# rhymes-ai/Aria

Measured on NVIDIA H100. Metric: Aria-25.3B bf16 prefill tokens/sec, higher is better.
Workload: dtype bf16

## Files before the change

### aria_b200/csrc/gemm.cu

```cuda
#include <cuda_fp8.h>

#include "gemm_common.cuh"

namespace aria {

constexpr int GEMM_STAGES = 4;
constexpr int FP8_LAND_STAGES = 3;
constexpr int FP8_CONVERT_WARPS = 3;
constexpr int PAIR_MIN_ROWS = 2048;
template <int BN, bool B_FP8 = false>
constexpr int gemm_smem_bytes() {
  return 1024  + GEMM_STAGES * (A_STAGE_BYTES + BN * BK * 2) + BM * acc_ld(BN) * 4 + 256  +
         (B_FP8 ? FP8_LAND_STAGES * BN * BK : 0);
}
static_assert(gemm_smem_bytes<128, true>() <= 232448, "fp8 landing ring must fit the opt-in shared memory of a block");

ARIA_DEVICE void e4m3x16_to_bf16(const uint4 v, uint4& lo, uint4& hi) {
  const uint32_t w[4] = {v.x, v.y, v.z, v.w};
  uint32_t o[8];
#pragma unroll
  for (int i = 0; i < 4; ++i) {
#pragma unroll
    for (int h = 0; h < 2; ++h) {
      const __half2_raw hr = __nv_cvt_fp8x2_to_halfraw2(static_cast<__nv_fp8x2_storage_t>(w[i] >> (16 * h)), __NV_E4M3);
      const float2 f = __half22float2(__half2(hr));
      o[2 * i + h] = pack_bf16(f.x, f.y);
    }
  }
  lo = make_uint4(o[0], o[1], o[2], o[3]);
  hi = make_uint4(o[4], o[5], o[6], o[7]);
}

template <bool PAIR> ARIA_DEVICE int first_tile() { return PAIR ? blockIdx.x >> 1 : blockIdx.x; }
template <bool PAIR> ARIA_DEVICE int tile_step() { return PAIR ? gridDim.x >> 1 : gridDim.x; }
template <bool PAIR> ARIA_DEVICE int pair_sched_n(int n_tiles) { return PAIR ? (n_tiles + 1) / 2 : n_tiles; }

template <int BN, bool B_MN>
ARIA_DEVICE void wgmma_tile_k16(float (&acc)[BN / 2], uint64_t da, uint64_t db) {
  if constexpr (BN == 128) wgmma_m64n128_ss<0, B_MN ? 1 : 0>(acc, da, db, 1u);
  else wgmma_m64n144_ss<0, B_MN ? 1 : 0>(acc, da, db, 1u);
}

template <int BN, bool B_MN, int EPI, bool B_FP8 = false, bool PAIR = false>
__global__ void __launch_bounds__(GEMM_THREADS, 1)
gemm_kernel(const __grid_constant__ CUtensorMap tmA, const __grid_constant__ CUtensorMap tmB0,
            const __grid_constant__ CUtensorMap tmB1, const __grid_constant__ CUtensorMap tmB2, const GemmParams p) {
  constexpr int B_STAGE_BYTES = BN * BK * 2;
  constexpr int STAGE_BYTES = A_STAGE_BYTES + B_STAGE_BYTES;
  constexpr int STAGES = GEMM_STAGES;
  constexpr int ACC_LD = acc_ld(BN);
  constexpr int OUT_BN = (EPI == ARIA_EPI_SWIGLU) ? BN / 2 : BN;
  static_assert(BN == 128 || BN == 144, "tile widths with a wgmma wrapper");
  static_assert(!B_FP8 || (B_MN && BN == 128 && EPI != ARIA_EPI_HEADS), "fp8 B: grouped [G, K, N] weights, 128-wide tiles");
  static_assert(!PAIR || (!B_MN && !B_FP8), "CTA pairs: dense K-major bf16 B");
  constexpr int LAND_BYTES = BN * BK;

  uint8_t* smem = smem_1024();
  float* stg = reinterpret_cast<float*>(smem + STAGES * STAGE_BYTES);
  const BarrierRing<STAGES> bar(stg + BM * ACC_LD);
  const BarrierRing<FP8_LAND_STAGES> land_bar(bar.empty + STAGES);
  uint8_t* land = reinterpret_cast<uint8_t*>(bar.full) + 256;

  const int warp = threadIdx.x >> 5;
  const int lane = threadIdx.x & 31;
  const int wg = threadIdx.x >> 7;

  if (warp == 0 && lane == 0) {
    prefetch_tmap(&tmA);
    prefetch_tmap(&tmB0);
    if (p.n_seg > 1 || EPI == ARIA_EPI_SWIGLU) prefetch_tmap(&tmB1);
    if (p.n_seg > 2) prefetch_tmap(&tmB2);
    bar.init(B_FP8 ? 1 + FP8_CONVERT_WARPS : 1, PAIR ? 2 * CONSUMER_WARPS : CONSUMER_WARPS);
    if constexpr (B_FP8) land_bar.init(1, FP8_CONVERT_WARPS);
    fence_mbar_init();
  }
  if constexpr (PAIR) cluster_sync();
  else __syncthreads();

  const int n_out_total = p.N * (EPI == ARIA_EPI_SWIGLU ? 1 : p.n_seg);
  const int n_tiles = (n_out_total + OUT_BN - 1) / OUT_BN;
  const int k_blocks = (p.K + BK - 1) / BK;
  const uint32_t smem_base = smem_u32(smem);
  const uint32_t full0 = smem_u32(bar.full), empty0 = smem_u32(bar.empty);

  if (wg == 0) {
    setmaxnreg_dec<40>();
    if (warp == 0 && elect_one()) {
      const uint32_t rank = PAIR ? cluster_ctarank() : 0;
      TileSched sched;
      sched.init(p, pair_sched_n<PAIR>(n_tiles));
      RingPos<STAGES> rp;
      RingPos<FP8_LAND_STAGES> lp;
      for (int t = first_tile<PAIR>();; t += tile_step<PAIR>()) {
        int grp, m_idx, n_idx, row0, rows;
        if (!sched.decode(t, grp, m_idx, n_idx, row0, rows)) break;
        if constexpr (PAIR) n_idx = 2 * n_idx + rank;
        const bool phantom = PAIR && n_idx >= n_tiles;
        const int a_row = row0 + m_idx * BM;
        const int a_half_row = a_row + (m_idx * BM + static_cast<int>(rank) * (BM / 2) < rows ? rank * (BM / 2) : 0);
        const int bgrp = weight_block(p, grp);
        int b_c0 = 0, b_c1 = 0;
        const CUtensorMap* tb0 = &tmB0;
        const CUtensorMap* tb1 = &tmB1;
        if constexpr (B_MN) {
          b_c0 = bgrp * p.K;
        } else if constexpr (EPI == ARIA_EPI_SWIGLU) {
          b_c0 = b_c1 = n_idx * OUT_BN;
        } else {
          const int col = n_idx * BN;
          const int seg = col / p.N;
          tb0 = seg == 0 ? &tmB0 : (seg == 1 ? &tmB1 : &tmB2);
          b_c0 = col - seg * p.N + bgrp * p.b_group_rows;
        }
        for (int kb = 0; kb < k_blocks; ++kb) {
          const uint32_t fb = full0 + rp.stage * 8;
          const uint32_t sa = smem_base + rp.stage * STAGE_BYTES;
          const uint32_t sb = sa + A_STAGE_BYTES;
          mbar_wait_addr(empty0 + rp.stage * 8, rp.phase ^ 1);
          if constexpr (PAIR) {
            mbar_arrive_expect_tx_addr(fb, phantom ? A_STAGE_BYTES : STAGE_BYTES);
            tma_load_2d_multicast_addr(sa + rank * (A_STAGE_BYTES / 2), &tmA, fb, kb * BK, a_half_row, 0b11);
            if (phantom) {
              rp.next();
              continue;
            }
          } else {
            mbar_arrive_expect_tx_addr(fb, B_FP8 ? A_STAGE_BYTES : STAGE_BYTES);
            tma_load_2d_addr(sa, &tmA, fb, kb * BK, a_row);
          }
          if constexpr (B_MN) {
            uint32_t dst = sb, box_bytes = 64 * BK * 2, bar_addr = fb;
            if constexpr (B_FP8) {
              bar_addr = smem_u32(land_bar.full) + lp.stage * 8;
              mbar_wait_addr(smem_u32(land_bar.empty) + lp.stage * 8, lp.phase ^ 1);
              mbar_arrive_expect_tx_addr(bar_addr, LAND_BYTES);
              dst = smem_u32(land) + lp.stage * LAND_BYTES;
              box_bytes = 64 * BK;
            }
            const int krow = b_c0 + kb * BK;
#pragma unroll
            for (int c = 0; c < BN / 64; ++c)
              tma_load_2d_addr(dst + c * box_bytes, &tmB0, bar_addr, tile_b_col<BN, EPI>(c * 64, n_idx, p.N), krow);
            if constexpr (B_FP8) lp.next();
          } else if constexpr (EPI == ARIA_EPI_SWIGLU) {
            tma_load_2d_addr(sb, tb0, fb, kb * BK, b_c0);
            tma_load_2d_addr(sb + (BN / 2) * BK * 2, tb1, fb, kb * BK, b_c1);
          } else {
            tma_load_2d_addr(sb, tb0, fb, kb * BK, b_c0);
          }
          rp.next();
        }
      }
    } else if constexpr (B_FP8) {
      if (warp > 0) {
        const int ct = threadIdx.x - 32;
        TileSched sched;
        sched.init(p, n_tiles);
        RingPos<STAGES> rp;
        RingPos<FP8_LAND_STAGES> lp;
        for (int t = blockIdx.x;; t += gridDim.x) {
          int grp, m_idx, n_idx, row0, rows;
          if (!sched.decode(t, grp, m_idx, n_idx, row0, rows)) break;
          for (int kb = 0; kb < k_blocks; ++kb) {
            mbar_wait_addr(smem_u32(land_bar.full) + lp.stage * 8, lp.phase);
            const uint8_t* src = land + lp.stage * LAND_BYTES;
            uint8_t* dst = smem + rp.stage * STAGE_BYTES + A_STAGE_BYTES;
#pragma unroll 1
            for (int i = ct; i < LAND_BYTES / 16; i += FP8_CONVERT_WARPS * 32) {
              const uint4 v = *reinterpret_cast<const uint4*>(src + i * 16);
              uint4 lo, hi;
              e4m3x16_to_bf16(v, lo, hi);
              const int r = (i >> 2) & 63, j = 2 * (i & 3);
              uint8_t* row = dst + (i >> 8) * (64 * BK * 2) + r * 128;
              *reinterpret_cast<uint4*>(row + ((j ^ (r & 7)) << 4)) = lo;
              *reinterpret_cast<uint4*>(row + (((j + 1) ^ (r & 7)) << 4)) = hi;
            }
            fence_proxy_async_smem();
            __syncwarp();
            if (lane == 0) {
              mbar_arrive(&bar.full[rp.stage]);
              mbar_arrive(&land_bar.empty[lp.stage]);
            }
            rp.next();
            lp.next();
          }
        }
      }
    }
  } else {
    setmaxnreg_inc<232>();
    const int cw = wg - 1;
    constexpr uint32_t b_lbo = B_MN ? 64 * BK * 2 : 16;
    constexpr uint32_t b_sbo = 1024;
    constexpr uint32_t b_kadv = (B_MN ? 16 * 128 : 32) >> 4;
    const uint64_t da0 = make_smem_desc(smem_base + cw * 64 * 128, 16, 1024);
    const uint64_t db0 = make_smem_desc(smem_base + A_STAGE_BYTES, b_lbo, b_sbo);
    const ConsumerThread ct = consumer_thread(cw, lane);
    const uint32_t rank = PAIR ? cluster_ctarank() : 0;
    TileSched sched;
    sched.init(p, pair_sched_n<PAIR>(n_tiles));
    RingPos<STAGES> rp;
    auto release = [&](int s) {
      if (lane == 0) {
        mbar_arrive(&bar.empty[s]);
        if constexpr (PAIR) mbar_arrive_cluster(&bar.empty[s], rank ^ 1);
      }
    };
    for (int t = first_tile<PAIR>();; t += tile_step<PAIR>()) {
      int grp, m_idx, n_idx, row0, rows;
      if (!sched.decode(t, grp, m_idx, n_idx, row0, rows)) break;
      if constexpr (PAIR) {
        n_idx = 2 * n_idx + rank;
        if (n_idx >= n_tiles) {
          for (int kb = 0; kb < k_blocks; ++kb) {
            mbar_wait_addr(full0 + rp.stage * 8, rp.phase);
            release(rp.stage);
            rp.next();
          }
          continue;
        }
      }
      float acc[BN / 2];
#pragma unroll
      for (int i = 0; i < BN / 2; ++i) acc[i] = 0.f;
      float2 bsc[BN / 8];
      if constexpr (B_FP8) load_col_scales<BN, EPI>(p, grp, n_idx, ct.frag_col, bsc);
      int prev = -1;
      for (int kb = 0; kb < k_blocks; ++kb) {
        mbar_wait_addr(full0 + rp.stage * 8, rp.phase);
        const uint64_t da = da0 + rp.stage * (STAGE_BYTES >> 4);
        const uint64_t db = db0 + rp.stage * (STAGE_BYTES >> 4);
        wgmma_fence();
#pragma unroll
        for (int k = 0; k < BK / 16; ++k) wgmma_tile_k16<BN, B_MN>(acc, da + k * 2, db + k * b_kadv);
        wgmma_commit();
        wgmma_wait<1>();
        if (prev >= 0) release(prev);
        prev = static_cast<int>(rp.stage);
        rp.next();
      }
      wgmma_wait<0>();
      fence_regs(acc);
      if (prev >= 0) release(prev);
      stage_and_epilogue<BN, EPI, B_FP8 ? AccScale::COL : AccScale::NONE>(p, stg, ct, acc, bsc, 1.f, 1.f, n_out_total, grp,
                                                                           m_idx, n_idx, row0, rows);
    }
  }
  if constexpr (PAIR) cluster_sync();
}

constexpr int W8_BK = 128;
static_assert(BM * W8_BK == A_STAGE_BYTES, "W8A8 A stage = bf16 A stage");

template <int EPI>
__global__ void __launch_bounds__(GEMM_THREADS, 1)
gemm_w8a8_kernel(const __grid_constant__ CUtensorMap tmA, const __grid_constant__ CUtensorMap tmB, const GemmParams p,
                 const float* __restrict__ a_scale) {
  constexpr int BN = 128;
  constexpr int STAGE_BYTES = A_STAGE_BYTES + BN * W8_BK;
  constexpr int STAGES = GEMM_STAGES;
  constexpr int ACC_LD = acc_ld(BN);
  constexpr int OUT_BN = (EPI == ARIA_EPI_SWIGLU) ? BN / 2 : BN;
  static_assert(EPI == ARIA_EPI_LINEAR || EPI == ARIA_EPI_SWIGLU, "W8A8: expert GEMM epilogues");

  uint8_t* smem = smem_1024();
  float* stg = reinterpret_cast<float*>(smem + STAGES * STAGE_BYTES);
  const BarrierRing<STAGES> bar(stg + BM * ACC_LD);

  const int warp = threadIdx.x >> 5;
  const int lane = threadIdx.x & 31;
  const int wg = threadIdx.x >> 7;

  if (warp == 0 && lane == 0) {
    prefetch_tmap(&tmA);
    prefetch_tmap(&tmB);
    bar.init(1, CONSUMER_WARPS);
    fence_mbar_init();
  }
  __syncthreads();

  const int n_tiles = (p.N + OUT_BN - 1) / OUT_BN;
  const int k_blocks = p.K / W8_BK;
  const uint32_t smem_base = smem_u32(smem);
  const uint32_t full0 = smem_u32(bar.full), empty0 = smem_u32(bar.empty);

  if (wg == 0) {
    setmaxnreg_dec<40>();
    if (warp == 0 && elect_one()) {
      TileSched sched;
      sched.init(p, n_tiles);
      RingPos<STAGES> rp;
      for (int t = blockIdx.x;; t += gridDim.x) {
        int grp, m_idx, n_idx, row0, rows;
        if (!sched.decode(t, grp, m_idx, n_idx, row0, rows)) break;
        const int a_row = row0 + m_idx * BM;
        int b_r0, b_r1;
        if constexpr (EPI == ARIA_EPI_SWIGLU) {
          b_r0 = weight_block(p, grp) * 2 * p.N + n_idx * OUT_BN;
          b_r1 = b_r0 + p.N;
        } else {
          b_r0 = weight_block(p, grp) * p.N + n_idx * BN;
          b_r1 = b_r0 + 64;
        }
        for (int kb = 0; kb < k_blocks; ++kb) {
          const uint32_t fb = full0 + rp.stage * 8;
          const uint32_t sa = smem_base + rp.stage * STAGE_BYTES;
          const uint32_t sb = sa + A_STAGE_BYTES;
          mbar_wait_addr(empty0 + rp.stage * 8, rp.phase ^ 1);
          mbar_arrive_expect_tx_addr(fb, STAGE_BYTES);
          tma_load_2d_addr(sa, &tmA, fb, kb * W8_BK, a_row);
          tma_load_2d_addr(sb, &tmB, fb, kb * W8_BK, b_r0);
          tma_load_2d_addr(sb + 64 * W8_BK, &tmB, fb, kb * W8_BK, b_r1);
          rp.next();
        }
      }
    }
  } else {
    setmaxnreg_inc<232>();
    const int cw = wg - 1;
    const uint64_t da0 = make_smem_desc(smem_base + cw * 64 * 128, 16, 1024);
    const uint64_t db0 = make_smem_desc(smem_base + A_STAGE_BYTES, 16, 1024);
    const ConsumerThread ct = consumer_thread(cw, lane);
    TileSched sched;
    sched.init(p, n_tiles);
    RingPos<STAGES> rp;
    float part[BN / 2];
    for (int t = blockIdx.x;; t += gridDim.x) {
      int grp, m_idx, n_idx, row0, rows;
// ... 53 lines not shown
  p.ldo = d->ldo;
  p.head_dim = d->head_dim;
  p.head_ld = d->head_ld;
  p.rows_per_batch = d->rows_per_batch > 0 ? d->rows_per_batch : static_cast<int>(d->m);
  p.pos0 = d->pos0;
  p.stride_b = d->stride_b;
  p.stride_h = d->stride_h;
  p.rope_mask = d->rope_mask;
  p.rope_cos = static_cast<const __nv_bfloat16*>(d->rope_cos);
  p.rope_sin = static_cast<const __nv_bfloat16*>(d->rope_sin);
  p.position_ids = d->position_ids;
  p.b_scale = b_scale;
  return p;
}

static aria_gemm_desc_t grouped_desc(const void* a, const void* b, void* out, const int32_t* offsets, int64_t rows, int64_t k,
                                     int64_t n, int32_t groups, int32_t epilogue) {
  aria_gemm_desc_t d{};
  d.a = a;
  d.lda = k;
  d.m = rows;
  d.n = n;
  d.k = k;
  d.b[0] = b;
  d.n_seg = 1;
  d.b_layout = ARIA_B_GKN;
  d.num_groups = groups;
  d.group_offsets = offsets;
  d.epilogue = epilogue;
  d.out[0] = out;
  d.ldo = n;
  return d;
}

static int64_t max_tiles(const aria_gemm_desc_t* d, int BN, int64_t groups) {
  const bool swiglu = d->epilogue == ARIA_EPI_SWIGLU;
  const int out_bn = swiglu ? BN / 2 : BN;
  const int64_t n_out_total = d->n * (swiglu ? 1 : d->n_seg);
  return (n_out_total + out_bn - 1) / out_bn * ((d->m + BM - 1) / BM + groups);
}

static int gemm_run(const aria_gemm_desc_t* d, const float* b_scale, cudaStream_t stream) {
  ARIA_CHECK_ARG(d != nullptr);
  ARIA_CHECK_ARG(d->a && d->b[0] && d->out[0]);
  ARIA_CHECK_ARG(d->m >= 0 && d->n > 0 && d->k > 0);
  ARIA_CHECK_ARG(d->n % 8 == 0 && d->k % 8 == 0 && d->lda % 8 == 0);
  ARIA_CHECK_ARG(d->n_seg >= 1 && d->n_seg <= 3);
  ARIA_CHECK_ARG(d->num_groups >= 1 && (d->group_mod >= 0 || d->num_groups % (-d->group_mod) == 0));
  ARIA_CHECK_ARG((reinterpret_cast<uintptr_t>(d->a) & 15) == 0 && (reinterpret_cast<uintptr_t>(d->out[0]) & 15) == 0);
  if (d->m == 0) return ARIA_OK;
  const bool b_mn = d->b_layout == ARIA_B_GKN;
  const bool b_gnk = d->b_layout == ARIA_B_GNK;
  const bool swiglu = d->epilogue == ARIA_EPI_SWIGLU;
  if (b_mn) {
    ARIA_CHECK_ARG(d->n_seg == 1);
    ARIA_CHECK_ARG(d->k % BK == 0 || (d->num_groups == 1 && d->group_mod == 0));
    ARIA_CHECK_ARG(d->n % 64 == 0);
    ARIA_CHECK_ARG(d->epilogue != ARIA_EPI_HEADS);
  } else {
    ARIA_CHECK_ARG(d->num_groups == 1 || d->n_seg == 1);
    if (swiglu) ARIA_CHECK_ARG(d->n_seg == 2 && d->b[1]);
    if (b_gnk) ARIA_CHECK_ARG(d->n_seg == 1 && !swiglu && d->epilogue == ARIA_EPI_LINEAR && d->n % 128 == 0);
    else ARIA_CHECK_ARG(d->num_groups == 1);
  }
  if (d->num_groups > 1) ARIA_CHECK_ARG(d->group_offsets != nullptr);
  if (d->group_counts) ARIA_CHECK_ARG(d->group_offsets != nullptr);
  if (d->out_group_base) ARIA_CHECK_ARG(d->out_group_row0 != nullptr && d->epilogue == ARIA_EPI_LINEAR && d->group_offsets != nullptr);
  ARIA_CHECK_ARG(d->a_rows == 0 || d->a_rows >= d->m);

  int BN = 128;
  if (d->epilogue == ARIA_EPI_HEADS) {
    ARIA_CHECK_ARG(d->head_dim > 0 && d->head_dim % 8 == 0 && d->head_ld >= d->head_dim && d->n % d->head_dim == 0);
    if (d->rope_mask) ARIA_CHECK_ARG(d->head_dim == 128 && d->rope_cos && d->rope_sin);
    if (d->n % 128 != 0) {
      ARIA_CHECK_ARG(!d->rope_mask && d->n % 144 == 0);
      BN = 144;
    }
    for (int s = 0; s < d->n_seg; ++s) ARIA_CHECK_ARG(d->out[s] && d->b[s]);
  } else {
    if (swiglu) ARIA_CHECK_ARG(d->n % 64 == 0);
    if (d->n_seg > 1 && !swiglu) ARIA_CHECK_ARG(d->n % BN == 0);
  }

  const bool pair = !b_scale && d->b_layout == ARIA_B_NK && d->num_groups == 1 && !d->group_offsets &&
                    d->epilogue == ARIA_EPI_LINEAR && d->m >= PAIR_MIN_ROWS;

  CUtensorMap tmA, tmB[3];
  int rc = make_tmap_2d(&tmA, d->a, d->k, d->a_rows > 0 ? d->a_rows : d->m, d->lda * 2, BK, pair ? BM / 2 : BM);
  if (rc) return rc;
  if (b_mn) {
    const uint64_t ncols = swiglu ? 2 * d->n : d->n;
    const uint64_t n_weights = d->group_mod > 0 ? d->group_mod : (d->group_mod < 0 ? d->num_groups / (-d->group_mod) : d->num_groups);
    rc = b_scale ? make_tmap_2d(&tmB[0], d->b[0], ncols, n_weights * d->k, ncols, 64, BK, CU_TENSOR_MAP_SWIZZLE_NONE,
                                CU_TENSOR_MAP_DATA_TYPE_UINT8)
                 : make_tmap_2d(&tmB[0], d->b[0], ncols, n_weights * d->k, ncols * 2, 64, BK);
    if (rc) return rc;
    tmB[1] = tmB[0];
    tmB[2] = tmB[0];
  } else {
    const int nb = swiglu ? 2 : d->n_seg;
    const uint32_t box_rows = swiglu ? BN / 2 : BN;
    for (int s = 0; s < 3; ++s) {
      const void* ptr = s < nb ? d->b[s] : d->b[0];
      const uint64_t b_rows = b_gnk ? static_cast<uint64_t>(d->group_mod > 0 ? d->group_mod : (d->group_mod < 0 ? d->num_groups / (-d->group_mod) : d->num_groups)) * d->n : d->n;
      rc = make_tmap_2d(&tmB[s], ptr, d->k, b_rows, d->k * 2, BK, box_rows);
      if (rc) return rc;
    }
  }

  const GemmParams p = gemm_params(d, b_scale);
  const int64_t tiles = max_tiles(d, BN, d->num_groups > 1 ? d->num_groups : 0);
  if (pair) {
    const int64_t m_tiles = (d->m + BM - 1) / BM, pairs = (tiles / m_tiles + 1) / 2 * m_tiles;
    return launch_persistent_pairs<gemm_kernel<128, false, ARIA_EPI_LINEAR, false, true>>(
        "gemm_kernel", GEMM_THREADS, gemm_smem_bytes<128>(), pairs, stream, tmA, tmB[0], tmB[1], tmB[2], p);
  }
#define ARIA_LAUNCH(BN_, MN_, EPI_, ...)                                                                                     \
  return launch_persistent<gemm_kernel<BN_, MN_, EPI_, ##__VA_ARGS__>>("gemm_kernel", GEMM_THREADS,                          \
                                                                       gemm_smem_bytes<BN_, ##__VA_ARGS__>(), tiles, stream, \
                                                                       tmA, tmB[0], tmB[1], tmB[2], p)
  if (b_scale) {
    if (swiglu) ARIA_LAUNCH(128, true, ARIA_EPI_SWIGLU, true);
    ARIA_LAUNCH(128, true, ARIA_EPI_LINEAR, true);
  }
  if (d->epilogue == ARIA_EPI_HEADS) {
    if (BN == 128) ARIA_LAUNCH(128, false, ARIA_EPI_HEADS);
    ARIA_LAUNCH(144, false, ARIA_EPI_HEADS);
  }
  if (swiglu) {
    if (b_mn) ARIA_LAUNCH(128, true, ARIA_EPI_SWIGLU);
    ARIA_LAUNCH(128, false, ARIA_EPI_SWIGLU);
  }
  if (b_mn) ARIA_LAUNCH(128, true, ARIA_EPI_LINEAR);
  ARIA_LAUNCH(128, false, ARIA_EPI_LINEAR);
#undef ARIA_LAUNCH
}

extern "C" int aria_gemm(const aria_gemm_desc_t* d, aria_stream_t stream) {
  return gemm_run(d, nullptr, reinterpret_cast<cudaStream_t>(stream));
}

int aria::grouped_gemm(const void* a, const void* b, const float* b_scale, void* out, const int32_t* offsets, int64_t rows,
                       int64_t k, int64_t n, int32_t groups, int32_t epilogue, cudaStream_t stream) {
  const aria_gemm_desc_t d = grouped_desc(a, b, out, offsets, rows, k, n, groups, epilogue);
  return gemm_run(&d, b_scale, stream);
}

extern "C" int aria_grouped_gemm(const void* a, const void* b, void* out, const int32_t* group_offsets, int64_t rows,
                                 int64_t k, int64_t n, int32_t num_groups, aria_stream_t stream) {
  return grouped_gemm(a, b, nullptr, out, group_offsets, rows, k, n, num_groups, ARIA_EPI_LINEAR,
                      reinterpret_cast<cudaStream_t>(stream));
}

extern "C" int aria_grouped_gemm_fp8(const void* a, const void* b_fp8, const float* b_scale, void* out,
                                     const int32_t* group_offsets, int64_t rows, int64_t k, int64_t n, int32_t num_groups,
                                     int32_t epilogue, aria_stream_t stream) {
  ARIA_CHECK_ARG(a && b_fp8 && b_scale && out && group_offsets);
  ARIA_CHECK_ARG(rows >= 0 && k > 0 && n > 0 && k % BK == 0 && n % 64 == 0 && num_groups >= 1);
  ARIA_CHECK_ARG(epilogue == ARIA_EPI_LINEAR || epilogue == ARIA_EPI_SWIGLU);
  ARIA_CHECK_ARG((reinterpret_cast<uintptr_t>(a) & 15) == 0 && (reinterpret_cast<uintptr_t>(b_fp8) & 15) == 0 &&
                 (reinterpret_cast<uintptr_t>(b_scale) & 15) == 0 && (reinterpret_cast<uintptr_t>(out) & 15) == 0);
  return grouped_gemm(a, b_fp8, b_scale, out, group_offsets, rows, k, n, num_groups, epilogue,
                      reinterpret_cast<cudaStream_t>(stream));
}

extern "C" int aria_grouped_gemm_w8a8(const void* a_fp8, const float* a_scale, const void* b_fp8_nk, const float* b_scale,
                                      void* out, const int32_t* group_offsets, int64_t rows, int64_t k, int64_t n,
                                      int32_t num_groups, int32_t epilogue, aria_stream_t stream_) {
  ARIA_CHECK_ARG(a_fp8 && a_scale && b_fp8_nk && b_scale && out && group_offsets);
  ARIA_CHECK_ARG(rows >= 0 && rows < (int64_t(1) << 31) && k > 0 && n > 0 && k % W8_BK == 0 && n % 64 == 0 && num_groups >= 1);
  ARIA_CHECK_ARG(k <= (1 << 30) && n <= (1 << 29) && static_cast<int64_t>(num_groups) * n * 2 < (int64_t(1) << 31));
  ARIA_CHECK_ARG(epilogue == ARIA_EPI_LINEAR || epilogue == ARIA_EPI_SWIGLU);
  ARIA_CHECK_ARG((reinterpret_cast<uintptr_t>(a_fp8) & 15) == 0 && (reinterpret_cast<uintptr_t>(b_fp8_nk) & 15) == 0 &&
                 (reinterpret_cast<uintptr_t>(b_scale) & 15) == 0 && (reinterpret_cast<uintptr_t>(out) & 15) == 0 &&
                 (reinterpret_cast<uintptr_t>(a_scale) & 3) == 0);
  if (rows == 0) return ARIA_OK;
  const bool swiglu = epilogue == ARIA_EPI_SWIGLU;
  const aria_gemm_desc_t d = grouped_desc(a_fp8, b_fp8_nk, out, group_offsets, rows, k, n, num_groups, epilogue);
  const GemmParams p = gemm_params(&d, b_scale);

  CUtensorMap tmA, tmB;
  int rc = make_tmap_2d(&tmA, a_fp8, k, rows, k, W8_BK, BM, CU_TENSOR_MAP_SWIZZLE_128B, CU_TENSOR_MAP_DATA_TYPE_UINT8);
  if (rc) return rc;
  rc = make_tmap_2d(&tmB, b_fp8_nk, k, num_groups * (swiglu ? 2 * n : n), k, W8_BK, 64, CU_TENSOR_MAP_SWIZZLE_128B,
                    CU_TENSOR_MAP_DATA_TYPE_UINT8);
  if (rc) return rc;

  const int64_t tiles = max_tiles(&d, 128, num_groups);
  constexpr int SMEM = gemm_smem_bytes<128>();
  cudaStream_t stream = reinterpret_cast<cudaStream_t>(stream_);
  if (swiglu)
    return launch_persistent<gemm_w8a8_kernel<ARIA_EPI_SWIGLU>>("gemm_w8a8_kernel", GEMM_THREADS, SMEM, tiles, stream, tmA,
                                                                 tmB, p, a_scale);
  return launch_persistent<gemm_w8a8_kernel<ARIA_EPI_LINEAR>>("gemm_w8a8_kernel", GEMM_THREADS, SMEM, tiles, stream, tmA, tmB,
                                                              p, a_scale);
}

extern "C" int aria_abi_version(void) { return 3; }
extern "C" const char* aria_build_arch(void) { return "sm_90a"; }
```

### aria_b200/csrc/gemm_common.cuh

```cuda
#pragma once
#include "common.cuh"
#include "ptx.cuh"

namespace aria {

constexpr int BM = 128;
constexpr int BK = 64;
constexpr int A_STAGE_BYTES = BM * BK * 2;
constexpr int GEMM_THREADS = 384;
constexpr int CONSUMER_WARPS = 8;
constexpr int acc_ld(int BN) { return BN + 4; }

struct GemmParams {
  int M, N, K;
  int num_groups;
  const int32_t* group_offsets;
  const int32_t* group_counts;
  const uint64_t* out_group_base;
  const int32_t* out_group_row0;
  int b_group_rows;
  int group_mod;
  int n_seg;
  int act;
  const __nv_bfloat16* bias[3];
// ... 260 lines not shown
    constexpr int NHC = BN / 64;
#pragma unroll 1
    for (int hc = half * NHC / 2; hc < (half ? NHC : NHC / 2); hc += 1) {
      const int hh = hc >> 1, c = (hc & 1) * 32;
      __nv_bfloat16* orow = obase + (cseg0 / p.head_dim + hh) * p.stride_h;
      const float* th = acc + hh * 128;
      uint32_t lo[32], hi[32];
      ld_acc32(th + c, lo);
      ld_acc32(th + 64 + c, hi);
      uint4 tc_lo[4], ts_lo[4], tc_hi[4], ts_hi[4];
#pragma unroll
      for (int q = 0; q < 4; ++q) {
        tc_lo[q] = __ldg(reinterpret_cast<const uint4*>(cs + c + q * 8));
        ts_lo[q] = __ldg(reinterpret_cast<const uint4*>(sn + c + q * 8));
        tc_hi[q] = __ldg(reinterpret_cast<const uint4*>(cs + 64 + c + q * 8));
        ts_hi[q] = __ldg(reinterpret_cast<const uint4*>(sn + 64 + c + q * 8));
      }
      if (row_ok) {
#pragma unroll
        for (int q = 0; q < 4; ++q) {
          const uint4 c_lo = tc_lo[q], s_lo = ts_lo[q], c_hi = tc_hi[q], s_hi = ts_hi[q];
          const uint32_t cl[4] = {c_lo.x, c_lo.y, c_lo.z, c_lo.w}, sl[4] = {s_lo.x, s_lo.y, s_lo.z, s_lo.w};
          const uint32_t ch[4] = {c_hi.x, c_hi.y, c_hi.z, c_hi.w}, sh[4] = {s_hi.x, s_hi.y, s_hi.z, s_hi.w};
          float ol[8], oh[8];
#pragma unroll
          for (int j = 0; j < 8; ++j) {
            float xl = __uint_as_float(lo[q * 8 + j]);
            float xh = __uint_as_float(hi[q * 8 + j]);
            bf16r2(xl, xh);
            float cosl = (j & 1) ? bf16_hi(cl[j >> 1]) : bf16_lo(cl[j >> 1]);
            float sinl = (j & 1) ? bf16_hi(sl[j >> 1]) : bf16_lo(sl[j >> 1]);
            float cosh_ = (j & 1) ? bf16_hi(ch[j >> 1]) : bf16_lo(ch[j >> 1]);
            float sinh_ = (j & 1) ? bf16_hi(sh[j >> 1]) : bf16_lo(sh[j >> 1]);
            float a0 = xl * cosl, a1 = -xh * sinl, b0 = xh * cosh_, b1 = xl * sinh_;
            bf16r2(a0, a1);
            bf16r2(b0, b1);
            ol[j] = a0 + a1;
            oh[j] = b0 + b1;
          }
          *reinterpret_cast<uint4*>(orow + c + q * 8) =
              make_uint4(pack_bf16(ol[0], ol[1]), pack_bf16(ol[2], ol[3]), pack_bf16(ol[4], ol[5]), pack_bf16(ol[6], ol[7]));
          *reinterpret_cast<uint4*>(orow + 64 + c + q * 8) =
              make_uint4(pack_bf16(oh[0], oh[1]), pack_bf16(oh[2], oh[3]), pack_bf16(oh[4], oh[5]), pack_bf16(oh[6], oh[7]));
        }
      }
    }
  }
}

template <int BN>
ARIA_DEVICE void heads_store_tile(const GemmParams& p, const float* stg, int cw, int m_idx, int n_idx, int row0, int rows) {
  constexpr int ACC_LD = acc_ld(BN), CH = BN / 8;
  const int col0 = n_idx * BN;
  const int seg = col0 / p.N;
  const int cseg0 = col0 - seg * p.N;
  const __nv_bfloat16* bias = p.bias[seg];
  __nv_bfloat16* out = p.out[seg];
#pragma unroll 1
  for (int i = threadIdx.x & 127; i < 64 * CH; i += 128) {
    const int r = cw * 64 + i / CH, c = (i % CH) * 8;
    const int r_in_grp = m_idx * BM + r;
    const int cs = cseg0 + c;
    if (r_in_grp >= rows || cs + 8 > p.N) continue;
    const float4 lo = *reinterpret_cast<const float4*>(stg + r * ACC_LD + c);
    const float4 hi = *reinterpret_cast<const float4*>(stg + r * ACC_LD + c + 4);
    float x[8] = {lo.x, lo.y, lo.z, lo.w, hi.x, hi.y, hi.z, hi.w};
    if (bias) {
      const uint4 bv = __ldg(reinterpret_cast<const uint4*>(bias + cs));
      const uint32_t bw[4] = {bv.x, bv.y, bv.z, bv.w};
#pragma unroll
      for (int j = 0; j < 4; ++j) {
        x[2 * j] += bf16_lo(bw[j]);
        x[2 * j + 1] += bf16_hi(bw[j]);
      }
    }
    const int grow = row0 + r_in_grp;
    const int b = grow / p.rows_per_batch, tok = grow - b * p.rows_per_batch;
    const int head = cs / p.head_dim, d = cs - head * p.head_dim;
    *reinterpret_cast<uint4*>(out + b * p.stride_b + static_cast<int64_t>(p.pos0 + tok) * p.head_ld + head * p.stride_h + d) =
        make_uint4(pack_bf16(x[0], x[1]), pack_bf16(x[2], x[3]), pack_bf16(x[4], x[5]), pack_bf16(x[6], x[7]));
  }
}

enum class AccScale { NONE, COL, ROW_COL };

template <int BN, int EPI, AccScale SCALE>
ARIA_DEVICE void stage_and_epilogue(const GemmParams& p, float* stg, const ConsumerThread& ct, const float (&acc)[BN / 2],
                                    const float2 (&bsc)[BN / 8], float as0, float as1, int n_out_total, int grp, int m_idx,
                                    int n_idx, int row0, int rows) {
  constexpr int ACC_LD = acc_ld(BN);
  auto scaled = [](float a, float as, float bs) {
    if constexpr (SCALE == AccScale::ROW_COL) return a * as * bs;
    else if constexpr (SCALE == AccScale::COL) return a * bs;
    else return a;
  };
  named_bar_sync(1 + ct.cw, 128);
#pragma unroll
  for (int j = 0; j < BN / 8; ++j) {
    float* d0 = stg + ct.frag_row * ACC_LD + 8 * j + ct.frag_col;
    *reinterpret_cast<float2*>(d0) = make_float2(scaled(acc[4 * j], as0, bsc[j].x), scaled(acc[4 * j + 1], as0, bsc[j].y));
    *reinterpret_cast<float2*>(d0 + 8 * ACC_LD) =
        make_float2(scaled(acc[4 * j + 2], as1, bsc[j].x), scaled(acc[4 * j + 3], as1, bsc[j].y));
  }
  named_bar_sync(1 + ct.cw, 128);
  if constexpr (EPI == ARIA_EPI_HEADS) {
    if (!((p.rope_mask >> (n_idx * BN / p.N)) & 1)) {
      heads_store_tile<BN>(p, stg, ct.cw, m_idx, n_idx, row0, rows);
      return;
    }
  }
  const int r_in_grp = m_idx * BM + ct.epi_row;
  const bool row_ok = r_in_grp < rows;
  const int64_t grow = static_cast<int64_t>(row0) + r_in_grp;
  epilogue_tile<BN, EPI>(p, stg + ct.epi_row * ACC_LD, n_out_total, n_idx, grow, row_ok, ct.half, grp, r_in_grp);
}

}
```

### aria_b200/csrc/ptx.cuh

```cuda
#pragma once
#include <cuda.h>
#include <cuda_bf16.h>
#include <cuda_runtime.h>
#include <stdint.h>

namespace aria {

#define ARIA_DEVICE __device__ __forceinline__

ARIA_DEVICE uint32_t smem_u32(const void* p) { return static_cast<uint32_t>(__cvta_generic_to_shared(p)); }

ARIA_DEVICE uint32_t elect_one() {
  uint32_t pred = 0;
  asm volatile(
      "{\n\t.reg .pred P;\n\t"
      "elect.sync _|P, 0xffffffff;\n\t"
      "selp.b32 %0, 1, 0, P;\n\t}\n"
      : "=r"(pred));
  return pred;
}

ARIA_DEVICE void mbar_init(uint64_t* bar, uint32_t count) {
  asm volatile("mbarrier.init.shared::cta.b64 [%0], %1;" ::"r"(smem_u32(bar)), "r"(count));
}
ARIA_DEVICE void fence_mbar_init() { asm volatile("fence.mbarrier_init.release.cluster;" ::: "memory"); }
ARIA_DEVICE void fence_proxy_async_smem() { asm volatile("fence.proxy.async.shared::cta;" ::: "memory"); }

ARIA_DEVICE void mbar_arrive_expect_tx(uint64_t* bar, uint32_t bytes) {
  asm volatile("mbarrier.arrive.expect_tx.shared::cta.b64 _, [%0], %1;" ::"r"(smem_u32(bar)), "r"(bytes)
               : "memory");
}
ARIA_DEVICE void mbar_arrive(uint64_t* bar) {
  asm volatile("mbarrier.arrive.shared::cta.b64 _, [%0];" ::"r"(smem_u32(bar)) : "memory");
}
ARIA_DEVICE bool mbar_try_wait(uint64_t* bar, uint32_t parity) {
  uint32_t ok;
  asm volatile(
      "{\n\t.reg .pred P;\n\t"
      "mbarrier.try_wait.parity.shared::cta.b64 P, [%1], %2;\n\t"
      "selp.b32 %0, 1, 0, P;\n\t}\n"
      : "=r"(ok) : "r"(smem_u32(bar)), "r"(parity) : "memory");
  return ok != 0;
}
ARIA_DEVICE void mbar_wait_addr(uint32_t addr, uint32_t parity) {
  uint32_t ok = 0;
  long long t0 = 0;
  for (uint32_t spin = 0;; ++spin) {
    asm volatile(
        "{\n\t.reg .pred P;\n\t"
        "mbarrier.try_wait.parity.shared::cta.b64 P, [%1], %2;\n\t"
        "selp.b32 %0, 1, 0, P;\n\t}\n"
        : "=r"(ok) : "r"(addr), "r"(parity) : "memory");
    if (ok) return;
    if ((spin & 0xFFF) == 0xFFF) {
      const long long now = clock64();
      if (t0 == 0) t0 = now;
      if (now - t0 > 4000000000ll) __trap();
    }
  }
}
ARIA_DEVICE void mbar_wait(uint64_t* bar, uint32_t parity) { mbar_wait_addr(smem_u32(bar), parity); }
ARIA_DEVICE void mbar_arrive_expect_tx_addr(uint32_t bar_addr, uint32_t bytes) {
  asm volatile("mbarrier.arrive.expect_tx.shared::cta.b64 _, [%0], %1;" ::"r"(bar_addr), "r"(bytes) : "memory");
}
ARIA_DEVICE void mbar_arrive_cluster(uint64_t* bar, uint32_t cta) {
  asm volatile(
      "{\n\t.reg .b32 ra;\n\t"
      "mapa.shared::cluster.u32 ra, %0, %1;\n\t"
      "mbarrier.arrive.shared::cluster.b64 _, [ra];\n\t}\n" ::"r"(smem_u32(bar)), "r"(cta)
      : "memory");
}

ARIA_DEVICE uint32_t cluster_ctarank() {
  uint32_t r;
  asm volatile("mov.u32 %0, %%cluster_ctarank;" : "=r"(r));
  return r;
}
ARIA_DEVICE void cluster_sync() {
  asm volatile("barrier.cluster.arrive.release;\n\tbarrier.cluster.wait.acquire;" ::: "memory");
}

ARIA_DEVICE void tma_load_2d_addr(uint32_t dst, const CUtensorMap* m, uint32_t bar_addr, int c0, int c1) {
  asm volatile(
      "cp.async.bulk.tensor.2d.shared::cluster.global.mbarrier::complete_tx::bytes [%0], [%1, {%3, %4}], [%2];"
      ::"r"(dst), "l"(reinterpret_cast<uint64_t>(m)), "r"(bar_addr), "r"(c0), "r"(c1)
      : "memory");
}
ARIA_DEVICE void tma_load_2d_multicast_addr(uint32_t dst, const CUtensorMap* m, uint32_t bar_addr, int c0, int c1,
                                            uint16_t cta_mask) {
  asm volatile(
      "cp.async.bulk.tensor.2d.shared::cluster.global.mbarrier::complete_tx::bytes.multicast::cluster [%0], [%1, {%3, %4}], [%2], %5;"
      ::"r"(dst), "l"(reinterpret_cast<uint64_t>(m)), "r"(bar_addr), "r"(c0), "r"(c1), "h"(cta_mask)
      : "memory");
}
ARIA_DEVICE void prefetch_tmap(const CUtensorMap* m) {
  asm volatile("prefetch.tensormap [%0];" ::"l"(reinterpret_cast<uint64_t>(m)) : "memory");
}
ARIA_DEVICE void tma_load_2d(void* dst, const CUtensorMap* m, uint64_t* bar, int c0, int c1) {
  asm volatile(
      "cp.async.bulk.tensor.2d.shared::cluster.global.mbarrier::complete_tx::bytes [%0], [%1, {%3, %4}], [%2];"
      ::"r"(smem_u32(dst)), "l"(reinterpret_cast<uint64_t>(m)), "r"(smem_u32(bar)), "r"(c0), "r"(c1)
      : "memory");
}
ARIA_DEVICE void tma_load_3d(void* dst, const CUtensorMap* m, uint64_t* bar, int c0, int c1, int c2) {
  asm volatile(
      "cp.async.bulk.tensor.3d.shared::cluster.global.mbarrier::complete_tx::bytes [%0], [%1, {%3, %4, %5}], [%2];"
      ::"r"(smem_u32(dst)), "l"(reinterpret_cast<uint64_t>(m)), "r"(smem_u32(bar)), "r"(c0), "r"(c1), "r"(c2)
      : "memory");
}
ARIA_DEVICE void tma_load_4d(void* dst, const CUtensorMap* m, uint64_t* bar, int c0, int c1, int c2, int c3) {
  asm volatile(
      "cp.async.bulk.tensor.4d.shared::cluster.global.mbarrier::complete_tx::bytes [%0], [%1, {%3, %4, %5, %6}], [%2];"
      ::"r"(smem_u32(dst)), "l"(reinterpret_cast<uint64_t>(m)), "r"(smem_u32(bar)), "r"(c0), "r"(c1), "r"(c2),
      "r"(c3)
      : "memory");
}

ARIA_DEVICE uint64_t make_smem_desc(uint32_t smem_addr, uint32_t lbo_bytes, uint32_t sbo_bytes) {
  uint64_t d = 0;
  d |= static_cast<uint64_t>((smem_addr & 0x3FFFF) >> 4);
  d |= static_cast<uint64_t>((lbo_bytes >> 4) & 0x3FFF) << 16;
  d |= static_cast<uint64_t>((sbo_bytes >> 4) & 0x3FFF) << 32;
  d |= 1ull << 62;
  return d;
}
ARIA_DEVICE uint64_t make_smem_desc_sw32(uint32_t smem_addr, uint32_t sbo_bytes) {
  uint64_t d = 0;
  d |= static_cast<uint64_t>((smem_addr & 0x3FFFF) >> 4);
  d |= static_cast<uint64_t>(1) << 16;
  d |= static_cast<uint64_t>((sbo_bytes >> 4) & 0x3FFF) << 32;
  d |= 3ull << 62;
  return d;
}
ARIA_DEVICE void wgmma_fence() { asm volatile("wgmma.fence.sync.aligned;" ::: "memory"); }
ARIA_DEVICE void wgmma_commit() { asm volatile("wgmma.commit_group.sync.aligned;" ::: "memory"); }
template <int N> ARIA_DEVICE void wgmma_wait() { asm volatile("wgmma.wait_group.sync.aligned %0;" ::"n"(N) : "memory"); }
template <int R> ARIA_DEVICE void fence_regs(float (&d)[R]) {
#pragma unroll
  for (int i = 0; i < R; ++i) asm volatile("" : "+f"(d[i])::"memory");
}
ARIA_DEVICE void named_bar_sync(uint32_t id, uint32_t threads) { asm volatile("bar.sync %0, %1;" ::"r"(id), "r"(threads) : "memory"); }
ARIA_DEVICE void named_bar_arrive(uint32_t id, uint32_t threads) { asm volatile("bar.arrive %0, %1;" ::"r"(id), "r"(threads) : "memory"); }

template <int TA, int TB>
ARIA_DEVICE void wgmma_m64n128_ss(float (&d)[64], uint64_t da, uint64_t db, uint32_t scale_d) {
  asm volatile(
      "{\n\t.reg .pred p;\n\tsetp.ne.b32 p, %66, 0;\n\t"
      "wgmma.mma_async.sync.aligned.m64n128k16.f32.bf16.bf16 {%0, %1, %2, %3, %4, %5, %6, %7, %8, %9, %10, %11, %12, %13, %14, %15, %16, %17, %18, %19, %20, %21, %22, %23, %24, %25, %26, %27, %28, %29, %30, %31, %32, %33, %34, %35, %36, %37, %38, %39, %40, %41, %42, %43, %44, %45, %46, %47, %48, %49, %50, %51, %52, %53, %54, %55, %56, %57, %58, %59, %60, %61, %62, %63}, %64, %65, p, 1, 1, %67, %68;\n\t}\n"
      : "+f"(d[0]), "+f"(d[1]), "+f"(d[2]), "+f"(d[3]), "+f"(d[4]), "+f"(d[5]), "+f"(d[6]), "+f"(d[7]), "+f"(d[8]), "+f"(d[9]), "+f"(d[10]), "+f"(d[11]), "+f"(d[12]), "+f"(d[13]), "+f"(d[14]), "+f"(d[15]), "+f"(d[16]), "+f"(d[17]), "+f"(d[18]), "+f"(d[19]), "+f"(d[20]), "+f"(d[21]), "+f"(d[22]), "+f"(d[23]), "+f"(d[24]), "+f"(d[25]), "+f"(d[26]), "+f"(d[27]), "+f"(d[28]), "+f"(d[29]), "+f"(d[30]), "+f"(d[31]), "+f"(d[32]), "+f"(d[33]), "+f"(d[34]), "+f"(d[35]), "+f"(d[36]), "+f"(d[37]), "+f"(d[38]), "+f"(d[39]), "+f"(d[40]), "+f"(d[41]), "+f"(d[42]), "+f"(d[43]), "+f"(d[44]), "+f"(d[45]), "+f"(d[46]), "+f"(d[47]), "+f"(d[48]), "+f"(d[49]), "+f"(d[50]), "+f"(d[51]), "+f"(d[52]), "+f"(d[53]), "+f"(d[54]), "+f"(d[55]), "+f"(d[56]), "+f"(d[57]), "+f"(d[58]), "+f"(d[59]), "+f"(d[60]), "+f"(d[61]), "+f"(d[62]), "+f"(d[63])
      : "l"(da), "l"(db), "r"(scale_d), "n"(TA), "n"(TB));
}
template <int TA, int TB>
ARIA_DEVICE void wgmma_m64n64_ss(float (&d)[32], uint64_t da, uint64_t db, uint32_t scale_d) {
  asm volatile(
      "{\n\t.reg .pred p;\n\tsetp.ne.b32 p, %34, 0;\n\t"
      "wgmma.mma_async.sync.aligned.m64n64k16.f32.bf16.bf16 {%0, %1, %2, %3, %4, %5, %6, %7, %8, %9, %10, %11, %12, %13, %14, %15, %16, %17, %18, %19, %20, %21, %22, %23, %24, %25, %26, %27, %28, %29, %30, %31}, %32, %33, p, 1, 1, %35, %36;\n\t}\n"
      : "+f"(d[0]), "+f"(d[1]), "+f"(d[2]), "+f"(d[3]), "+f"(d[4]), "+f"(d[5]), "+f"(d[6]), "+f"(d[7]), "+f"(d[8]), "+f"(d[9]), "+f"(d[10]), "+f"(d[11]), "+f"(d[12]), "+f"(d[13]), "+f"(d[14]), "+f"(d[15]), "+f"(d[16]), "+f"(d[17]), "+f"(d[18]), "+f"(d[19]), "+f"(d[20]), "+f"(d[21]), "+f"(d[22]), "+f"(d[23]), "+f"(d[24]), "+f"(d[25]), "+f"(d[26]), "+f"(d[27]), "+f"(d[28]), "+f"(d[29]), "+f"(d[30]), "+f"(d[31])
      : "l"(da), "l"(db), "r"(scale_d), "n"(TA), "n"(TB));
}
template <int TA, int TB>
ARIA_DEVICE void wgmma_m64n144_ss(float (&d)[72], uint64_t da, uint64_t db, uint32_t scale_d) {
  asm volatile(
      "{\n\t.reg .pred p;\n\tsetp.ne.b32 p, %74, 0;\n\t"
      "wgmma.mma_async.sync.aligned.m64n144k16.f32.bf16.bf16 {%0, %1, %2, %3, %4, %5, %6, %7, %8, %9, %10, %11, %12, %13, %14, %15, %16, %17, %18, %19, %20, %21, %22, %23, %24, %25, %26, %27, %28, %29, %30, %31, %32, %33, %34, %35, %36, %37, %38, %39, %40, %41, %42, %43, %44, %45, %46, %47, %48, %49, %50, %51, %52, %53, %54, %55, %56, %57, %58, %59, %60, %61, %62, %63, %64, %65, %66, %67, %68, %69, %70, %71}, %72, %73, p, 1, 1, %75, %76;\n\t}\n"
      : "+f"(d[0]), "+f"(d[1]), "+f"(d[2]), "+f"(d[3]), "+f"(d[4]), "+f"(d[5]), "+f"(d[6]), "+f"(d[7]), "+f"(d[8]), "+f"(d[9]), "+f"(d[10]), "+f"(d[11]), "+f"(d[12]), "+f"(d[13]), "+f"(d[14]), "+f"(d[15]), "+f"(d[16]), "+f"(d[17]), "+f"(d[18]), "+f"(d[19]), "+f"(d[20]), "+f"(d[21]), "+f"(d[22]), "+f"(d[23]), "+f"(d[24]), "+f"(d[25]), "+f"(d[26]), "+f"(d[27]), "+f"(d[28]), "+f"(d[29]), "+f"(d[30]), "+f"(d[31]), "+f"(d[32]), "+f"(d[33]), "+f"(d[34]), "+f"(d[35]), "+f"(d[36]), "+f"(d[37]), "+f"(d[38]), "+f"(d[39]), "+f"(d[40]), "+f"(d[41]), "+f"(d[42]), "+f"(d[43]), "+f"(d[44]), "+f"(d[45]), "+f"(d[46]), "+f"(d[47]), "+f"(d[48]), "+f"(d[49]), "+f"(d[50]), "+f"(d[51]), "+f"(d[52]), "+f"(d[53]), "+f"(d[54]), "+f"(d[55]), "+f"(d[56]), "+f"(d[57]), "+f"(d[58]), "+f"(d[59]), "+f"(d[60]), "+f"(d[61]), "+f"(d[62]), "+f"(d[63]), "+f"(d[64]), "+f"(d[65]), "+f"(d[66]), "+f"(d[67]), "+f"(d[68]), "+f"(d[69]), "+f"(d[70]), "+f"(d[71])
      : "l"(da), "l"(db), "r"(scale_d), "n"(TA), "n"(TB));
}
ARIA_DEVICE void wgmma_m64n128k32_e4m3_ss(float (&d)[64], uint64_t da, uint64_t db, uint32_t scale_d) {
  asm volatile(
      "{\n\t.reg .pred p;\n\tsetp.ne.b32 p, %66, 0;\n\t"
      "wgmma.mma_async.sync.aligned.m64n128k32.f32.e4m3.e4m3 {%0, %1, %2, %3, %4, %5, %6, %7, %8, %9, %10, %11, %12, %13, %14, %15, %16, %17, %18, %19, %20, %21, %22, %23, %24, %25, %26, %27, %28, %29, %30, %31, %32, %33, %34, %35, %36, %37, %38, %39, %40, %41, %42, %43, %44, %45, %46, %47, %48, %49, %50, %51, %52, %53, %54, %55, %56, %57, %58, %59, %60, %61, %62, %63}, %64, %65, p, 1, 1;\n\t}\n"
      : "+f"(d[0]), "+f"(d[1]), "+f"(d[2]), "+f"(d[3]), "+f"(d[4]), "+f"(d[5]), "+f"(d[6]), "+f"(d[7]), "+f"(d[8]), "+f"(d[9]), "+f"(d[10]), "+f"(d[11]), "+f"(d[12]), "+f"(d[13]), "+f"(d[14]), "+f"(d[15]), "+f"(d[16]), "+f"(d[17]), "+f"(d[18]), "+f"(d[19]), "+f"(d[20]), "+f"(d[21]), "+f"(d[22]), "+f"(d[23]), "+f"(d[24]), "+f"(d[25]), "+f"(d[26]), "+f"(d[27]), "+f"(d[28]), "+f"(d[29]), "+f"(d[30]), "+f"(d[31]), "+f"(d[32]), "+f"(d[33]), "+f"(d[34]), "+f"(d[35]), "+f"(d[36]), "+f"(d[37]), "+f"(d[38]), "+f"(d[39]), "+f"(d[40]), "+f"(d[41]), "+f"(d[42]), "+f"(d[43]), "+f"(d[44]), "+f"(d[45]), "+f"(d[46]), "+f"(d[47]), "+f"(d[48]), "+f"(d[49]), "+f"(d[50]), "+f"(d[51]), "+f"(d[52]), "+f"(d[53]), "+f"(d[54]), "+f"(d[55]), "+f"(d[56]), "+f"(d[57]), "+f"(d[58]), "+f"(d[59]), "+f"(d[60]), "+f"(d[61]), "+f"(d[62]), "+f"(d[63])
      : "l"(da), "l"(db), "r"(scale_d));
}
template <int TB>
ARIA_DEVICE void wgmma_m64n128_rs(float (&d)[64], const uint32_t (&a)[4], uint64_t db) {
  asm volatile(
// ... 57 lines not shown
```

Before: 17780.

## Add TMA-store register epilogue with prefetched residual for dense linear GEMMs

For dense bf16 K-major LINEAR GEMMs, the consumer warpgroups now convert accumulators to bf16 straight into a swizzled, double-buffered shared tile. They add bias, activation and a residual that TMA prefetches during the mainloop, then write the tile back with TMA bulk stores. This replaces the fp32 staging buffer and the generic stage_and_epilogue path, aiming to cut epilogue latency and global store traffic and to overlap stores with the next tile. It adds more barriers, alignment requirements on ldo/ldr/residual, and extra tensor maps in every kernel signature.

```diff
diff --git a/aria_b200/csrc/gemm.cu b/aria_b200/csrc/gemm.cu
--- a/aria_b200/csrc/gemm.cu
+++ b/aria_b200/csrc/gemm.cu
@@ -8,9 +8,13 @@
 constexpr int FP8_LAND_STAGES = 3;
 constexpr int FP8_CONVERT_WARPS = 3;
 constexpr int PAIR_MIN_ROWS = 2048;
-template <int BN, bool B_FP8 = false>
+template <int BN, bool TMA_EPI>
+constexpr int epi_smem_bytes() {
+  return TMA_EPI ? 2 * 2 * OUT_TILE_BYTES : BM * acc_ld(BN) * 4;
+}
+template <int BN, bool B_FP8 = false, bool TMA_EPI = false>
 constexpr int gemm_smem_bytes() {
-  return 1024  + GEMM_STAGES * (A_STAGE_BYTES + BN * BK * 2) + BM * acc_ld(BN) * 4 + 256  +
+  return 1024  + GEMM_STAGES * (A_STAGE_BYTES + BN * BK * 2) + epi_smem_bytes<BN, TMA_EPI>() + 256  +
          (B_FP8 ? FP8_LAND_STAGES * BN * BK : 0);
 }
 static_assert(gemm_smem_bytes<128, true>() <= 232448, "fp8 landing ring must fit the opt-in shared memory of a block");
@@ -41,25 +45,28 @@
   else wgmma_m64n144_ss<0, B_MN ? 1 : 0>(acc, da, db, 1u);
 }
 
-template <int BN, bool B_MN, int EPI, bool B_FP8 = false, bool PAIR = false>
+template <int BN, bool B_MN, int EPI, bool B_FP8 = false, bool PAIR = false, bool TMA_EPI = false>
 __global__ void __launch_bounds__(GEMM_THREADS, 1)
 gemm_kernel(const __grid_constant__ CUtensorMap tmA, const __grid_constant__ CUtensorMap tmB0,
-            const __grid_constant__ CUtensorMap tmB1, const __grid_constant__ CUtensorMap tmB2, const GemmParams p) {
+            const __grid_constant__ CUtensorMap tmB1, const __grid_constant__ CUtensorMap tmB2,
+            const __grid_constant__ CUtensorMap tmOut, const __grid_constant__ CUtensorMap tmRes, const GemmParams p) {
   constexpr int B_STAGE_BYTES = BN * BK * 2;
   constexpr int STAGE_BYTES = A_STAGE_BYTES + B_STAGE_BYTES;
   constexpr int STAGES = GEMM_STAGES;
-  constexpr int ACC_LD = acc_ld(BN);
   constexpr int OUT_BN = (EPI == ARIA_EPI_SWIGLU) ? BN / 2 : BN;
   static_assert(BN == 128 || BN == 144, "tile widths with a wgmma wrapper");
   static_assert(!B_FP8 || (B_MN && BN == 128 && EPI != ARIA_EPI_HEADS), "fp8 B: grouped [G, K, N] weights, 128-wide tiles");
-  static_assert(!PAIR || (!B_MN && !B_FP8), "CTA pairs: dense K-major bf16 B");
+  static_assert(!PAIR || TMA_EPI, "CTA pairs: dense LINEAR, register epilogue");
+  static_assert(!TMA_EPI || (!B_MN && !B_FP8 && BN == 128 && EPI == ARIA_EPI_LINEAR), "register epilogue: dense LINEAR");
   constexpr int LAND_BYTES = BN * BK;
 
   uint8_t* smem = smem_1024();
-  float* stg = reinterpret_cast<float*>(smem + STAGES * STAGE_BYTES);
-  const BarrierRing<STAGES> bar(stg + BM * ACC_LD);
+  uint8_t* epi = smem + STAGES * STAGE_BYTES;
+  float* stg = reinterpret_cast<float*>(epi);
+  const BarrierRing<STAGES> bar(epi + epi_smem_bytes<BN, TMA_EPI>());
   const BarrierRing<FP8_LAND_STAGES> land_bar(bar.empty + STAGES);
   uint8_t* land = reinterpret_cast<uint8_t*>(bar.full) + 256;
+  uint64_t* res_bar = bar.full + 16;
 
   const int warp = threadIdx.x >> 5;
   const int lane = threadIdx.x & 31;
@@ -72,6 +79,11 @@
     if (p.n_seg > 2) prefetch_tmap(&tmB2);
     bar.init(B_FP8 ? 1 + FP8_CONVERT_WARPS : 1, PAIR ? 2 * CONSUMER_WARPS : CONSUMER_WARPS);
     if constexpr (B_FP8) land_bar.init(1, FP8_CONVERT_WARPS);
+    if constexpr (TMA_EPI) {
+      prefetch_tmap(&tmOut);
+      if (p.residual) prefetch_tmap(&tmRes);
+      for (int i = 0; i < 4; ++i) mbar_init(&res_bar[i], 1);
+    }
     fence_mbar_init();
   }
   if constexpr (PAIR) cluster_sync();
@@ -200,6 +212,8 @@
     TileSched sched;
     sched.init(p, pair_sched_n<PAIR>(n_tiles));
     RingPos<STAGES> rp;
+    const bool lead = (threadIdx.x & 127) == 0;
+    uint32_t n_stored = 0, res_phase = 0;
     auto release = [&](int s) {
       if (lane == 0) {
         mbar_arrive(&bar.empty[s]);
@@ -225,6 +239,24 @@
       for (int i = 0; i < BN / 2; ++i) acc[i] = 0.f;
       float2 bsc[BN / 8];
       if constexpr (B_FP8) load_col_scales<BN, EPI>(p, grp, n_idx, ct.frag_col, bsc);
+      const int wg_row = row0 + m_idx * BM + cw * 64;
+      const bool live = m_idx * BM + cw * 64 < rows;
+      const uint32_t buf = n_stored & 1;
+      uint8_t* ot = epi + (2 * cw + buf) * OUT_TILE_BYTES;
+      uint32_t bw[BN / 8];
+      const __nv_bfloat16* bias = nullptr;
+      if constexpr (TMA_EPI) {
+        if (lead) {
+          bulk_wait_read<1>();
+          if (p.residual && live) {
+            const uint32_t rb = smem_u32(&res_bar[2 * cw + buf]);
+            const int boxes = n_idx * BN + 64 < n_out_total ? 2 : 1;
+            mbar_arrive_expect_tx_addr(rb, boxes * OUT_BOX_BYTES);
+            for (int b = 0; b < boxes; ++b) tma_load_2d_addr(smem_u32(ot) + b * OUT_BOX_BYTES, &tmRes, rb, n_idx * BN + 64 * b, wg_row);
+          }
+        }
+        bias = load_col_bias<BN>(p, n_out_total, n_idx, ct.frag_col, bw);
+      }
       int prev = -1;
       for (int kb = 0; kb < k_blocks; ++kb) {
         mbar_wait_addr(full0 + rp.stage * 8, rp.phase);
@@ -242,8 +274,29 @@
       wgmma_wait<0>();
       fence_regs(acc);
       if (prev >= 0) release(prev);
-      stage_and_epilogue<BN, EPI, B_FP8 ? AccScale::COL : AccScale::NONE>(p, stg, ct, acc, bsc, 1.f, 1.f, n_out_total, grp,
-                                                                           m_idx, n_idx, row0, rows);
+      if constexpr (TMA_EPI) {
+        if (!live) continue;
+        named_bar_sync(1 + cw, 128);
+        if (p.residual) {
+          mbar_wait(&res_bar[2 * cw + buf], (res_phase >> buf) & 1);
+          res_phase ^= 1u << buf;
+        }
+        linear_fragment_epilogue<BN>(p, ct, acc, bw, bias != nullptr, ot);
+        fence_proxy_async_smem();
+        named_bar_sync(1 + cw, 128);
+        if (lead) {
+          for (int b = 0; b < 2 && n_idx * BN + 64 * b < n_out_total; ++b)
+            tma_store_2d_addr(&tmOut, smem_u32(ot) + b * OUT_BOX_BYTES, n_idx * BN + 64 * b, wg_row);
+          bulk_commit();
+        }
+        ++n_stored;
+      } else {
+        stage_and_epilogue<BN, EPI, B_FP8 ? AccScale::COL : AccScale::NONE>(p, stg, ct, acc, bsc, 1.f, 1.f, n_out_total, grp,
+                                                                             m_idx, n_idx, row0, rows);
+      }
+    }
+    if constexpr (TMA_EPI) {
+      if (lead) bulk_wait<0>();
     }
   }
   if constexpr (PAIR) cluster_sync();
@@ -463,10 +516,14 @@
     if (d->n_seg > 1 && !swiglu) ARIA_CHECK_ARG(d->n % BN == 0);
   }
 
-  const bool pair = !b_scale && d->b_layout == ARIA_B_NK && d->num_groups == 1 && !d->group_offsets &&
-                    d->epilogue == ARIA_EPI_LINEAR && d->m >= PAIR_MIN_ROWS;
-
-  CUtensorMap tmA, tmB[3];
+  const int64_t n_out_total = swiglu ? d->n : d->n * d->n_seg;
+  const bool tma_epi = !b_scale && d->b_layout == ARIA_B_NK && d->num_groups == 1 && !d->group_offsets &&
+                       d->epilogue == ARIA_EPI_LINEAR && d->ldo % 8 == 0 && d->ldo >= n_out_total &&
+                       (!d->residual || (d->ldr % 8 == 0 && d->ldr >= n_out_total &&
+                                         (reinterpret_cast<uintptr_t>(d->residual) & 15) == 0));
+  const bool pair = tma_epi && d->m >= PAIR_MIN_ROWS;
+
+  CUtensorMap tmA, tmB[3], tmOut, tmRes;
   int rc = make_tmap_2d(&tmA, d->a, d->k, d->a_rows > 0 ? d->a_rows : d->m, d->lda * 2, BK, pair ? BM / 2 : BM);
   if (rc) return rc;
   if (b_mn) {
@@ -488,18 +545,32 @@
       if (rc) return rc;
     }
   }
+  tmOut = tmRes = tmA;
+  if (tma_epi) {
+    rc = make_tmap_2d(&tmOut, d->out[0], n_out_total, d->m, d->ldo * 2, 64, 64);
+    if (rc) return rc;
+    if (d->residual) {
+      rc = make_tmap_2d(&tmRes, d->residual, n_out_total, d->m, d->ldr * 2, 64, 64);
+      if (rc) return rc;
+    }
+  }
 
   const GemmParams p = gemm_params(d, b_scale);
   const int64_t tiles = max_tiles(d, BN, d->num_groups > 1 ? d->num_groups : 0);
   if (pair) {
     const int64_t m_tiles = (d->m + BM - 1) / BM, pairs = (tiles / m_tiles + 1) / 2 * m_tiles;
-    return launch_persistent_pairs<gemm_kernel<128, false, ARIA_EPI_LINEAR, false, true>>(
-        "gemm_kernel", GEMM_THREADS, gemm_smem_bytes<128>(), pairs, stream, tmA, tmB[0], tmB[1], tmB[2], p);
-  }
+    return launch_persistent_pairs<gemm_kernel<128, false, ARIA_EPI_LINEAR, false, true, true>>(
+        "gemm_kernel", GEMM_THREADS, gemm_smem_bytes<128, false, true>(), pairs, stream, tmA, tmB[0], tmB[1], tmB[2], tmOut,
+        tmRes, p);
+  }
+  if (tma_epi)
+    return launch_persistent<gemm_kernel<128, false, ARIA_EPI_LINEAR, false, false, true>>(
+        "gemm_kernel", GEMM_THREADS, gemm_smem_bytes<128, false, true>(), tiles, stream, tmA, tmB[0], tmB[1], tmB[2], tmOut,
+        tmRes, p);
 #define ARIA_LAUNCH(BN_, MN_, EPI_, ...)                                                                                     \
   return launch_persistent<gemm_kernel<BN_, MN_, EPI_, ##__VA_ARGS__>>("gemm_kernel", GEMM_THREADS,                          \
                                                                        gemm_smem_bytes<BN_, ##__VA_ARGS__>(), tiles, stream, \
-                                                                       tmA, tmB[0], tmB[1], tmB[2], p)
+                                                                       tmA, tmB[0], tmB[1], tmB[2], tmOut, tmRes, p)
   if (b_scale) {
     if (swiglu) ARIA_LAUNCH(128, true, ARIA_EPI_SWIGLU, true);
     ARIA_LAUNCH(128, true, ARIA_EPI_LINEAR, true);
diff --git a/aria_b200/csrc/gemm_common.cuh b/aria_b200/csrc/gemm_common.cuh
--- a/aria_b200/csrc/gemm_common.cuh
+++ b/aria_b200/csrc/gemm_common.cuh
@@ -366,6 +366,55 @@
   }
 }
 
+constexpr int OUT_BOX_BYTES = 64 * 64 * 2;
+constexpr int OUT_TILE_BYTES = 2 * OUT_BOX_BYTES;
+
+template <int BN>
+ARIA_DEVICE const __nv_bfloat16* load_col_bias(const GemmParams& p, int n_out_total, int n_idx, int frag_col,
+                                               uint32_t (&bw)[BN / 8]) {
+  const int col0 = n_idx * BN;
+  const int seg = col0 / p.N;
+  const __nv_bfloat16* bias = p.bias[seg];
+#pragma unroll
+  for (int j = 0; j < BN / 8; ++j) {
+    const int col = col0 + 8 * j + frag_col;
+    bw[j] = (bias && col < n_out_total) ? __ldg(reinterpret_cast<const uint32_t*>(bias + (col - seg * p.N))) : 0u;
+  }
+  return bias;
+}
+
+template <int BN>
+ARIA_DEVICE void linear_fragment_epilogue(const GemmParams& p, const ConsumerThread& ct, const float (&acc)[BN / 2],
+                                          const uint32_t (&bw)[BN / 8], bool has_bias, uint8_t* ot) {
+  static_assert(BN == 128, "two 64-column boxes per tile");
+  const int r = ct.frag_row & 63;
+#pragma unroll
+  for (int j = 0; j < BN / 8; ++j) {
+    uint8_t* chunk = ot + (j >> 3) * OUT_BOX_BYTES + r * 128 + ((((j & 7) ^ (r & 7))) << 4) + ct.frag_col * 2;
+#pragma unroll
+    for (int h = 0; h < 2; ++h) {
+      uint32_t* dst = reinterpret_cast<uint32_t*>(chunk + h * 8 * 128);
+      float x0 = acc[4 * j + 2 * h], x1 = acc[4 * j + 2 * h + 1];
+      if (has_bias) {
+        x0 += bf16_lo(bw[j]);
+        x1 += bf16_hi(bw[j]);
+      }
+      x0 = bf16r(x0);
+      x1 = bf16r(x1);
+      if (p.act != ARIA_ACT_NONE) {
+        x0 = bf16r(act_apply(x0, p.act));
+        x1 = bf16r(act_apply(x1, p.act));
+      }
+      if (p.residual) {
+        const uint32_t rw = *dst;
+        x0 += bf16_lo(rw);
+        x1 += bf16_hi(rw);
+      }
+      *dst = pack_bf16(x0, x1);
+    }
+  }
+}
+
 enum class AccScale { NONE, COL, ROW_COL };
 
 template <int BN, int EPI, AccScale SCALE>
diff --git a/aria_b200/csrc/ptx.cuh b/aria_b200/csrc/ptx.cuh
--- a/aria_b200/csrc/ptx.cuh
+++ b/aria_b200/csrc/ptx.cuh
@@ -93,6 +93,14 @@
       ::"r"(dst), "l"(reinterpret_cast<uint64_t>(m)), "r"(bar_addr), "r"(c0), "r"(c1), "h"(cta_mask)
       : "memory");
 }
+ARIA_DEVICE void tma_store_2d_addr(const CUtensorMap* m, uint32_t src, int c0, int c1) {
+  asm volatile("cp.async.bulk.tensor.2d.global.shared::cta.bulk_group [%0, {%2, %3}], [%1];"
+               ::"l"(reinterpret_cast<uint64_t>(m)), "r"(src), "r"(c0), "r"(c1)
+               : "memory");
+}
+ARIA_DEVICE void bulk_commit() { asm volatile("cp.async.bulk.commit_group;" ::: "memory"); }
+template <int N> ARIA_DEVICE void bulk_wait_read() { asm volatile("cp.async.bulk.wait_group.read %0;" ::"n"(N) : "memory"); }
+template <int N> ARIA_DEVICE void bulk_wait() { asm volatile("cp.async.bulk.wait_group %0;" ::"n"(N) : "memory"); }
 ARIA_DEVICE void prefetch_tmap(const CUtensorMap* m) {
   asm volatile("prefetch.tensormap [%0];" ::"l"(reinterpret_cast<uint64_t>(m)) : "memory");
 }
```

Result: faster. 18170, median of 6 (+2.2%).
